# mic-rud/Learned-Compression-of-Point-Cloud-Geometry-and-Attributes

Hardware: AMD Instinct MI355X
Metric: encode+decode Mpoints/sec (higher is better)
Workload: dtype f32

## Files before the change

### learned-compression-of-point-cloud-geometry-and-attributes_amd/csrc/select.hip

```cpp
#include <stdlib.h>

#include "common.h"
#include "sort_small.h"

namespace pcc {

constexpr int TK_STRIDE = 264;
constexpr int TK_LDS_BATCHES = 16;

__device__ __forceinline__ uint32_t float_key(float v) {
    if (v != v) return 0xFFFFFFFFu;
    if (v == 0.0f) v = 0.0f;
    const uint32_t u = __float_as_uint(v);
    return (u & 0x80000000u) ? ~u : (u | 0x80000000u);
}

struct Key96 { uint32_t w[3]; };

__device__ __forceinline__ Key96 make_key(float logit, int4 c) {
    const uint64_t lo = ~pack_key(c.x, c.y, c.z, c.w);
    Key96 k;
    k.w[0] = float_key(logit);
    k.w[1] = (uint32_t)(lo >> 32);
    k.w[2] = (uint32_t)lo;
// ... 201 lines not shown

__global__ __launch_bounds__(256) void topk_write_mask(const float* __restrict__ logits, int ld,
                                                       const int32_t* __restrict__ coords, int64_t n, int nbatch,
                                                       const int32_t* __restrict__ state, uint8_t* __restrict__ mask) {
    const int64_t i = (int64_t)blockIdx.x * 256 + threadIdx.x;
    if (i >= n) return;
    const int4 c = reinterpret_cast<const int4*>(coords)[i];
    const int b = c.x;
    uint8_t m = 0;
    if (b >= 0 && b < nbatch) {
        const int32_t* st = state + (int64_t)b * TK_STRIDE;
        const int nb = st[2];
        if (nb <= 12) m = cmp_prefix(make_key(logits[i * ld], c), st, nb) >= 0 ? 1 : 0;
    }
    mask[i] = m;
}

constexpr int TK_SMALL_N = 32768;
__global__ __launch_bounds__(1024) void topk_small_kernel(const float* __restrict__ logits, int ld, const int32_t* __restrict__ coords, int n,
                                                          const int32_t* __restrict__ k, uint8_t* __restrict__ mask,
                                                          int32_t* __restrict__ state) {
    __shared__ int32_t st[8];
    __shared__ int h[256];
    __shared__ int total_s;
    const int t = threadIdx.x;
    if (t < 8) st[t] = 0;
    __syncthreads();
    if (t == 0) {
        const int kk = k[0];
        st[0] = kk;
        if (kk <= 0) { st[1] = 1; st[2] = 13; }
    }
    __syncthreads();
    for (int pass = 0; pass < 12; ++pass) {
        if (st[1]) break;
        if (t < 256) h[t] = 0;
        __syncthreads();
        const bool logit_only = pass < 4;
        for (int i = t; i < n; i += 1024) {
            const int4 c = logit_only ? make_int4(0, 0, 0, 0) : reinterpret_cast<const int4*>(coords)[i];
            if (c.x != 0) continue;
            const Key96 key = make_key(logits[(int64_t)i * ld], c);
            if (cmp_prefix(key, st, pass) != 0) continue;
            atomicAdd(&h[(key.w[pass >> 2] >> (8 * (3 - (pass & 3)))) & 0xFFu], 1);
        }
        __syncthreads();
        const int krem = st[0];
        int above = 0, mine = 0;
        if (t < 256) {
            mine = h[t];
            for (int j = t + 1; j < 256; ++j) above += h[j];
            if (t == 0) total_s = above + mine;
        }
        __syncthreads();
        if (pass == 0 && total_s <= krem) {
            if (t == 0) { st[1] = 1; st[2] = 0; }
        } else if (t < 256 && above < krem && krem <= above + mine) {
            const int word = pass >> 2, shift = 8 * (3 - (pass & 3));
            st[3 + word] = (int32_t)((uint32_t)st[3 + word] | ((uint32_t)t << shift));
            const int knew = krem - above;
            st[0] = knew;
            if (mine == knew || pass == 11) { st[1] = 1; st[2] = pass + 1; }
        }
        __syncthreads();
    }
    const int nb = st[2];
    for (int i = t; i < n; i += 1024) {
        const int4 c = reinterpret_cast<const int4*>(coords)[i];
        uint8_t m = 0;
        if (c.x == 0 && nb <= 12) m = cmp_prefix(make_key(logits[(int64_t)i * ld], c), st, nb) >= 0 ? 1 : 0;
        mask[i] = m;
    }
    for (int i = t; i < TK_STRIDE; i += 1024) state[i] = i < 8 ? st[i] : 0;
}

__global__ __launch_bounds__(256) void coords_to_keys(const int32_t* __restrict__ coords, int64_t n,
                                                      uint64_t* __restrict__ keys) {
    const int64_t i = (int64_t)blockIdx.x * 256 + threadIdx.x;
    if (i >= n) return;
    const int4 c = reinterpret_cast<const int4*>(coords)[i];
    keys[i] = pack_key(c.x, c.y, c.z, c.w);
}

__global__ __launch_bounds__(256) void mask_bit_counts_kernel(const uint32_t* __restrict__ row_mask, int64_t n,
                                                              uint32_t* __restrict__ counts) {
    __shared__ unsigned c[27];
    if (threadIdx.x < 27) c[threadIdx.x] = 0u;
    __syncthreads();
    unsigned mine[27];
#pragma unroll
    for (int b = 0; b < 27; ++b) mine[b] = 0u;
    for (int64_t i0 = (int64_t)blockIdx.x * 256; i0 < n; i0 += (int64_t)gridDim.x * 256) {
        const int64_t i = i0 + threadIdx.x;
        const uint32_t m = (i < n) ? row_mask[i] : 0u;
#pragma unroll
        for (int b = 0; b < 27; ++b) mine[b] += (unsigned)__popcll(__ballot((m >> b) & 1u));
    }
    if ((threadIdx.x & 63) == 0) {
#pragma unroll
        for (int b = 0; b < 27; ++b)
            if (mine[b]) atomicAdd(&c[b], mine[b]);
    }
    __syncthreads();
    if (threadIdx.x < 27 && c[threadIdx.x]) atomicAdd(&counts[threadIdx.x], c[threadIdx.x]);
}

__device__ __forceinline__ void order_bit_positions(const uint32_t* __restrict__ counts, int* pos_s) {
    if (threadIdx.x < 27) {
        const uint32_t mine = counts[threadIdx.x];
        int rank = 0;
        for (int b = 0; b < 27; ++b) {
            const uint32_t o = counts[b];
            rank += (o < mine || (o == mine && b < (int)threadIdx.x)) ? 1 : 0;
        }
        pos_s[threadIdx.x] = 26 - rank;
    }
    __syncthreads();
}

__device__ __forceinline__ uint32_t order_key_of(uint32_t m, const int* pos_s) {
    uint32_t key = 0u;
#pragma unroll
    for (int b = 0; b < 27; ++b) key |= ((m >> b) & 1u) << pos_s[b];
    return 0x7FFFFFFu - key;
}

__global__ __launch_bounds__(256) void order_keys32_kernel(const uint32_t* __restrict__ row_mask, int64_t n,
                                                           const uint32_t* __restrict__ counts, uint32_t* __restrict__ keys) {
    __shared__ int pos_s[27];
    order_bit_positions(counts, pos_s);
    const int64_t i = (int64_t)blockIdx.x * 256 + threadIdx.x;
    if (i >= n) return;
    const uint32_t m = row_mask[i] & 0x7FFFFFFu;
    keys[i] = order_key_of(m, pos_s);
}

__global__ __launch_bounds__(256) void order_keys64_kernel(const uint32_t* __restrict__ row_mask,
                                                           const int32_t* __restrict__ coords, int64_t n,
                                                           int block_log2, int ts, const uint32_t* __restrict__ counts,
                                                           uint64_t* __restrict__ keys) {
    __shared__ int pos_s[27];
    order_bit_positions(counts, pos_s);
    const int64_t i = (int64_t)blockIdx.x * 256 + threadIdx.x;
    if (i >= n) return;
    uint64_t key = order_key_of(row_mask[i] & 0x7FFFFFFu, pos_s);
    const int4 c = reinterpret_cast<const int4*>(coords)[i];
    const uint64_t bx = (uint64_t)(((c.y / ts) + 512) >> block_log2) & 0x3FF;
    const uint64_t by = (uint64_t)(((c.z / ts) + 512) >> block_log2) & 0x3FF;
    const uint64_t bz = (uint64_t)(((c.w / ts) + 512) >> block_log2) & 0x3FF;
    key |= ((((uint64_t)(c.x & 0x3) << 30) | (bx << 20) | (by << 10) | bz) << 32);
    keys[i] = key;
}

__global__ __launch_bounds__(256) void group_masks_kernel(const int32_t* __restrict__ order, const uint32_t* __restrict__ row_mask,
                                                          int64_t n, uint32_t* __restrict__ group_mask32) {
    const int64_t i = (int64_t)blockIdx.x * 256 + threadIdx.x;
    uint32_t m = (i < n) ? row_mask[order[i]] : 0u;
#pragma unroll
    for (int d = 1; d < 32; d <<= 1) m |= __shfl_xor(m, d, 64);
    if (i < n && (threadIdx.x & 31) == 0) group_mask32[i >> 5] = m;
}

__global__ __launch_bounds__(256) void permute_rows_kernel(const int32_t* __restrict__ order, const int32_t* __restrict__ nbr,
                                                           int64_t n, int K, int32_t* __restrict__ nbr_sorted) {
    __shared__ int32_t src_row[256];
    const int64_t r0 = (int64_t)blockIdx.x * 256;
    const int64_t i = r0 + threadIdx.x;
    src_row[threadIdx.x] = (i < n) ? order[i] : 0;
    __syncthreads();
    const int rows = (int)((n - r0 < 256) ? (n - r0) : 256);
    const int total = rows * K;
    int32_t* dst = nbr_sorted + r0 * K;
    for (int e = threadIdx.x; e < total; e += 256) {
        const int lr = e / K;
        const int k = e - lr * K;
        dst[e] = nbr[(int64_t)src_row[lr] * K + k];
    }
}


template <int ROUNDS>
__global__ __launch_bounds__(RS_SMALL_THREADS) void order_small_kernel(const uint32_t* __restrict__ row_mask, int n, uint32_t* keys_a,
                                                                      uint32_t* keys_b, int32_t* va, int32_t* vb) {
    __shared__ unsigned cnt27[27];
    __shared__ int pos_s[27];
    const int t = threadIdx.x;
    if (t < 27) cnt27[t] = 0u;
    __syncthreads();
    unsigned mine[27];
#pragma unroll
    for (int b = 0; b < 27; ++b) mine[b] = 0u;
    for (int i = t; i < n; i += RS_SMALL_THREADS) {
        const uint32_t m = row_mask[i];
#pragma unroll
        for (int b = 0; b < 27; ++b) mine[b] += (m >> b) & 1u;
    }
#pragma unroll
    for (int b = 0; b < 27; ++b) {
        unsigned v = mine[b];
#pragma unroll
        for (int d = 32; d >= 1; d >>= 1) v += __shfl_xor(v, d, 64);
        if ((t & 63) == 0 && v) atomicAdd(&cnt27[b], v);
    }
    __syncthreads();
    order_bit_positions(cnt27, pos_s);
    for (int i = t; i < n; i += RS_SMALL_THREADS) keys_a[i] = order_key_of(row_mask[i] & 0x7FFFFFFu, pos_s);
    __syncthreads();
    radix_sort_small_body<uint32_t, ROUNDS, 9>(keys_a, keys_b, va, vb, 1, n, 0, 27, 3);
}

constexpr int SMALL_MAP_MAX = 256;

template <int ROUNDS, int KS>
__global__ __launch_bounds__(RS_SMALL_THREADS) void small_map_kernel(const int32_t* __restrict__ out_coords, int n,
                                                                    const uint64_t* __restrict__ keys, const int32_t* __restrict__ vals,
                                                                    uint64_t tmask, int tshift, int step, int pitch,
                                                                    int32_t* nbr, uint32_t* __restrict__ row_mask, int32_t* order,
// ... 83 lines not shown
extern "C" {

int64_t pcc_small_map_max(void) {
    static int off = -1;
    if (off < 0) { const char* e = getenv("PCC_SMALL_MAP"); off = (e && e[0] == '0') ? 1 : 0; }
    return off ? 0 : SMALL_MAP_MAX;
}

int pcc_small_kernel_map(const int32_t* out_coords, int64_t n_out, const uint64_t* in_keys, const int32_t* in_vals, int64_t in_cap,
                         int32_t ksize, int32_t step, int32_t sign, int32_t* nbr, uint32_t* row_mask, int32_t* order,
                         uint32_t* group_mask32, void* scratch, int64_t scratch_bytes, void* stream) {
    PCC_REQUIRE(ksize == 2 || ksize == 3, "pcc_small_kernel_map: kernel size must be 2 or 3");
    PCC_REQUIRE(sign == 1 || sign == -1, "pcc_small_kernel_map: sign must be +1/-1");
    PCC_REQUIRE(in_cap > 0 && (in_cap & (in_cap - 1)) == 0, "pcc_small_kernel_map: bad capacity");
    PCC_REQUIRE(step >= 1, "pcc_small_kernel_map: step must be >= 1");
    PCC_REQUIRE(n_out >= 0 && n_out <= SMALL_MAP_MAX, "pcc_small_kernel_map: %lld rows exceed %d", (long long)n_out, SMALL_MAP_MAX);
    PCC_REQUIRE(scratch_bytes >= pcc_sort_scratch_bytes(n_out), "pcc_small_kernel_map: scratch too small");
    if (n_out <= 0) return PCC_OK;
    const int in_stride = sign > 0 ? step : 2 * step;
    const int pitch = sign > 0 ? 0 : 2 * step;
    char* p = reinterpret_cast<char*>(scratch);
    uint32_t* keys_a = reinterpret_cast<uint32_t*>(p); p += align256(n_out * 8);
    uint32_t* keys_b = reinterpret_cast<uint32_t*>(p); p += align256(n_out * 8);
    int32_t* vals_x = reinterpret_cast<int32_t*>(p);
    const int rounds = (int)(((n_out + RS_SMALL_WAVES - 1) / RS_SMALL_WAVES + 63) / 64);
    hipStream_t st = as_stream(stream);
#define PCC_SMALL_MAP(R, S)                                                                                                          \
    hipLaunchKernelGGL((small_map_kernel<R, S>), dim3(1), dim3(RS_SMALL_THREADS), 0, st, out_coords, (int)n_out, in_keys, in_vals,    \
                       (uint64_t)(in_cap - 1), grid_shift_of(in_stride), sign * step, pitch, nbr, row_mask, order,                   \
                       group_mask32, keys_a, keys_b, vals_x)
#define PCC_SMALL_MAP_R(S)                                                                                                           \
    do {                                                                                                                             \
        if (rounds <= 1) PCC_SMALL_MAP(1, S);                                                                                        \
        else if (rounds <= 2) PCC_SMALL_MAP(2, S);                                                                                   \
        else PCC_SMALL_MAP(4, S);                                                                                                    \
    } while (0)
    if (ksize == 3) PCC_SMALL_MAP_R(3);
    else PCC_SMALL_MAP_R(2);
#undef PCC_SMALL_MAP_R
#undef PCC_SMALL_MAP
    PCC_LAUNCH_CHECK();
    return PCC_OK;
}

int64_t pcc_topk_state_elems(int32_t nbatch) { return (int64_t)nbatch * TK_STRIDE + (nbatch == 1 ? (int64_t)TK1_GROUPS * 256 : 0); }

int pcc_topk_mask(const float* logits, int32_t ld, const int32_t* coords, int64_t n, int32_t nbatch, const int32_t* k,
                  uint8_t* mask, int32_t* state, void* stream) {
    PCC_REQUIRE(nbatch >= 1 && nbatch <= BATCH_LIMIT + 1, "pcc_topk_mask: bad nbatch %d", nbatch);
    PCC_REQUIRE(ld >= 1, "pcc_topk_mask: bad leading dimension");
    hipStream_t st = as_stream(stream);
    if (small_path_enabled(1) && nbatch == 1 && n > 0 && n <= TK_SMALL_N) {
        hipLaunchKernelGGL(topk_small_kernel, dim3(1), dim3(1024), 0, st, logits, ld, coords, (int)n, k, mask, state);
        PCC_LAUNCH_CHECK();
        return PCC_OK;
    }
    hipLaunchKernelGGL(topk_init, dim3(nbatch), dim3(256), 0, st, k, nbatch, state);
    if (n > 0) {
        const unsigned nb = blocks_for(n, 256, 512);
        if (nbatch == 1 && small_path_enabled(1)) {
            const unsigned groups = blocks_for(n, TK1_THREADS * 4, TK1_GROUPS);
            int32_t* partial = state + TK_STRIDE;
            for (int pass = 0; pass < 4; ++pass) {
                hipLaunchKernelGGL(topk_hist1_kernel, dim3(groups), dim3(TK1_THREADS), 0, st, logits, ld, n, pass, state, partial);
                hipLaunchKernelGGL(topk_pick1_kernel, dim3(1), dim3(1024), 0, st, pass, state, partial, (int)groups);
            }
            hipLaunchKernelGGL(topk_tail_kernel, dim3(1), dim3(1024), 0, st, logits, ld, coords, n, state);
            hipLaunchKernelGGL(topk_write_mask, dim3(blocks_for(n, 256)), dim3(256), 0, st, logits, ld, coords, n, nbatch,
                               state, mask);
            PCC_LAUNCH_CHECK();
            return PCC_OK;
        }
        for (int pass = 0; pass < 12; ++pass) {
            hipLaunchKernelGGL(topk_hist, dim3(nb), dim3(256), 0, st, logits, ld, coords, n, nbatch, pass, state);
            hipLaunchKernelGGL(topk_pick, dim3(nbatch), dim3(256), 0, st, pass, state);
        }
        hipLaunchKernelGGL(topk_write_mask, dim3(blocks_for(n, 256)), dim3(256), 0, st, logits, ld, coords, n, nbatch,
                           state, mask);
    }
    PCC_LAUNCH_CHECK();
    return PCC_OK;
}

int64_t pcc_order_scratch_bytes(int64_t n) { return pcc_sort_scratch_bytes(n); }

int pcc_order_rows_by_mask(const uint32_t* row_mask, const int32_t* coords, int64_t n, int32_t block_log2,
                           int32_t tensor_stride, int32_t* order, uint32_t* group_mask32, void* scratch, int64_t scratch_bytes,
                           void* stream) {
    if (n <= 0) return PCC_OK;
    PCC_REQUIRE(n < (1ll << 31), "pcc_order_rows_by_mask: too many rows");
    PCC_REQUIRE(block_log2 < 0 || coords != nullptr, "pcc_order_rows_by_mask: block ordering needs coordinates");
    PCC_REQUIRE(block_log2 <= 10, "pcc_order_rows_by_mask: block_log2 out of range");
    PCC_REQUIRE(tensor_stride >= 1, "pcc_order_rows_by_mask: bad tensor stride");
    PCC_REQUIRE(scratch_bytes >= pcc_sort_scratch_bytes(n), "pcc_order_rows_by_mask: scratch too small");
    hipStream_t st = as_stream(stream);
    char* p = reinterpret_cast<char*>(scratch);
    char* keys_a = p; p += align256(n * 8);
    char* keys_b = p; p += align256(n * 8);
    int32_t* vals_x = reinterpret_cast<int32_t*>(p); p += align256(n * 4);
    void* counters = p;
    uint32_t* bit_counts = reinterpret_cast<uint32_t*>(p + radix_sort_counter_bytes(n));
    if (small_path_enabled(0) && block_log2 < 0 && n <= RS_SMALL_N) {
        const int rounds = (int)(((n + RS_SMALL_WAVES - 1) / RS_SMALL_WAVES + 63) / 64);
        uint32_t* ka = reinterpret_cast<uint32_t*>(keys_a);
        uint32_t* kb = reinterpret_cast<uint32_t*>(keys_b);
#define PCC_ORDER_SMALL(R) hipLaunchKernelGGL(order_small_kernel<R>, dim3(1), dim3(RS_SMALL_THREADS), 0, st, row_mask, (int)n, ka, kb, vals_x, order)
        if (rounds <= 1) PCC_ORDER_SMALL(1);
        else if (rounds <= 2) PCC_ORDER_SMALL(2);
        else if (rounds <= 4) PCC_ORDER_SMALL(4);
        else if (rounds <= 8) PCC_ORDER_SMALL(8);
        else PCC_ORDER_SMALL(16);
#undef PCC_ORDER_SMALL
        hipLaunchKernelGGL(group_masks_kernel, dim3(blocks_for(n, 256)), dim3(256), 0, st, order, row_mask, n, group_mask32);
        PCC_LAUNCH_CHECK();
        return PCC_OK;
    }
    PCC_CHECK_HIP(hipMemsetAsync(bit_counts, 0, 27 * sizeof(uint32_t), st));
    hipLaunchKernelGGL(mask_bit_counts_kernel, dim3(blocks_for(n, 256 * 16, 512)), dim3(256), 0, st, row_mask, n, bit_counts);
    const int begin = 0, end = block_log2 >= 0 ? 64 : 27;
    const int digit_bits = block_log2 >= 0 ? 8 : radix_sort_order_digit_bits(n);
    const bool in_b = radix_sort_result_in_b(begin, end, digit_bits);
    int32_t* va = in_b ? vals_x : order;
    int32_t* vb = in_b ? order : vals_x;
    int rc;
    if (block_log2 < 0) {
        hipLaunchKernelGGL(order_keys32_kernel, dim3(blocks_for(n, 256)), dim3(256), 0, st, row_mask, n, bit_counts,
                           reinterpret_cast<uint32_t*>(keys_a));
        rc = radix_sort_pairs_u32(reinterpret_cast<uint32_t*>(keys_a), reinterpret_cast<uint32_t*>(keys_b), va, vb, true, n, begin, end,
                                  counters, st, digit_bits);
    } else {
        hipLaunchKernelGGL(order_keys64_kernel, dim3(blocks_for(n, 256)), dim3(256), 0, st, row_mask, coords, n, block_log2, tensor_stride,
                           bit_counts, reinterpret_cast<uint64_t*>(keys_a));
        rc = radix_sort_pairs_u64(reinterpret_cast<uint64_t*>(keys_a), reinterpret_cast<uint64_t*>(keys_b), va, vb, true, n, begin, end,
                                  counters, st);
    }
    if (rc) return rc;
    hipLaunchKernelGGL(group_masks_kernel, dim3(blocks_for(n, 256)), dim3(256), 0, st, order, row_mask, n, group_mask32);
    PCC_LAUNCH_CHECK();
    return PCC_OK;
}

int pcc_permute_map_rows(const int32_t* nbr, const int32_t* order, int64_t n, int32_t K, int32_t* nbr_sorted, void* stream) {
    PCC_REQUIRE(K >= 1 && K <= 27, "pcc_permute_map_rows: K out of range");
    PCC_REQUIRE(nbr != nullptr && order != nullptr && nbr_sorted != nullptr, "pcc_permute_map_rows: null argument");
    if (n <= 0) return PCC_OK;
    hipLaunchKernelGGL(permute_rows_kernel, dim3(blocks_for(n, 256)), dim3(256), 0, as_stream(stream), order, nbr, n, K, nbr_sorted);
    PCC_LAUNCH_CHECK();
    return PCC_OK;
}

int64_t pcc_sort_scratch_bytes(int64_t n) {
    if (n < 1) n = 1;
    return 2 * align256(n * 8) + align256(n * 4) + radix_sort_counter_bytes(n) + 256;
}

int pcc_sort_coords(const int32_t* coords, int64_t n, int32_t* perm, void* scratch, int64_t scratch_bytes, void* stream) {
    if (n <= 0) return PCC_OK;
    PCC_REQUIRE(n < (1ll << 31), "pcc_sort_coords: too many rows");
    PCC_REQUIRE(scratch_bytes >= pcc_sort_scratch_bytes(n), "pcc_sort_coords: scratch too small");
    hipStream_t st = as_stream(stream);
    char* p = reinterpret_cast<char*>(scratch);
    uint64_t* keys_a = reinterpret_cast<uint64_t*>(p); p += align256(n * 8);
    uint64_t* keys_b = reinterpret_cast<uint64_t*>(p); p += align256(n * 8);
    int32_t* vals_x = reinterpret_cast<int32_t*>(p); p += align256(n * 4);
    void* counters = p;
    hipLaunchKernelGGL(coords_to_keys, dim3(blocks_for(n, 256)), dim3(256), 0, st, coords, n, keys_a);
    const bool in_b = radix_sort_result_in_b(0, 64);
    return radix_sort_pairs_u64(keys_a, keys_b, in_b ? vals_x : perm, in_b ? perm : vals_x, true, n, 0, 64, counters, st);
}

}
```

### learned-compression-of-point-cloud-geometry-and-attributes_amd/csrc/sort.h

```cpp
#pragma once
#include "common.h"

namespace pcc {

static inline int64_t align256(int64_t v) { return (v + 255) / 256 * 256; }

int64_t scan_block_sums_elems(int64_t m);
int scan_flags(const int32_t* flags, int64_t m, int32_t* pos, int32_t* block_sums, int64_t* total, int inclusive,
               hipStream_t st, const int32_t* err = nullptr);

int radix_sort_passes(int begin_bit, int end_bit, int digit_bits = 8);
static inline bool radix_sort_result_in_b(int begin_bit, int end_bit, int digit_bits = 8) { return radix_sort_passes(begin_bit, end_bit, digit_bits) & 1; }
int64_t radix_sort_counter_bytes(int64_t n);
int radix_sort_order_digit_bits(int64_t n);
int radix_sort_pairs_u32(uint32_t* keys_a, uint32_t* keys_b, int32_t* vals_a, int32_t* vals_b, bool vals_are_iota, int64_t n,
                         int begin_bit, int end_bit, void* counters, hipStream_t st, int digit_bits = 8);
int radix_sort_pairs_u64(uint64_t* keys_a, uint64_t* keys_b, int32_t* vals_a, int32_t* vals_b, bool vals_are_iota, int64_t n,
                         int begin_bit, int end_bit, void* counters, hipStream_t st);

}
```

### learned-compression-of-point-cloud-geometry-and-attributes_amd/csrc/sort.hip

```cpp
#include "sort_small.h"

namespace pcc {

constexpr int RS_MID_ITEMS = 8;
constexpr int RS_MID_MAX_UNITS = 64;
constexpr int RS_BIG_ITEMS = 16;

template <class K, int ROUNDS, int DB>
__global__ __launch_bounds__(RS_SMALL_THREADS) void radix_sort_small_kernel(K* ka, K* kb, int32_t* va, int32_t* vb, int iota, int n,
                                                                           int begin_bit, int end_bit, int passes) {
    radix_sort_small_body<K, ROUNDS, DB>(ka, kb, va, vb, iota, n, begin_bit, end_bit, passes);
}

template <class K, int ITEMS, int DB>
__global__ __launch_bounds__(256) void radix_count_kernel(const K* __restrict__ keys, int64_t n, int shift, unsigned dmask,
                                                          int64_t nunits, int32_t* __restrict__ counts) {
    constexpr int ND = 1 << DB;
    __shared__ int cnt[ND];
#pragma unroll
    for (int d = threadIdx.x; d < ND; d += 256) cnt[d] = 0;
    __syncthreads();
    const int64_t base = (int64_t)blockIdx.x * (256 * ITEMS);
    K key[ITEMS];
#pragma unroll
    for (int j = 0; j < ITEMS; ++j) {
        const int64_t i = base + (int64_t)j * 256 + threadIdx.x;
        key[j] = (i < n) ? keys[i] : (K)0;
    }
#pragma unroll
    for (int j = 0; j < ITEMS; ++j)
        if (base + (int64_t)j * 256 + threadIdx.x < n) atomicAdd(&cnt[(unsigned)(key[j] >> shift) & dmask], 1);
    __syncthreads();
#pragma unroll
    for (int d = threadIdx.x; d < ND; d += 256) counts[(int64_t)d * nunits + blockIdx.x] = cnt[d];
}

__global__ __launch_bounds__(256) void radix_rowscan_kernel(int32_t* __restrict__ counts, int64_t nunits, int32_t* __restrict__ totals) {
    __shared__ int wsum[4];
    __shared__ int carry_s;
    const int t = threadIdx.x, lane = t & 63, w = t >> 6;
    int32_t* row = counts + (int64_t)blockIdx.x * nunits;
    if (t == 0) carry_s = 0;
    __syncthreads();
    for (int64_t base = 0; base < nunits; base += 1024) {
        const int64_t i = base + 4 * (int64_t)t;
        int f[4];
        int v = 0;
#pragma unroll
        for (int j = 0; j < 4; ++j) {
            f[j] = (i + j < nunits) ? row[i + j] : 0;
            v += f[j];
        }
        const int inc = wave_inclusive_scan_i32(v, lane);
        if (lane == 63) wsum[w] = inc;
        __syncthreads();
        int pre = carry_s;
        for (int ww = 0; ww < w; ++ww) pre += wsum[ww];
        int ex = pre + inc - v;
#pragma unroll
        for (int j = 0; j < 4; ++j) {
            if (i + j < nunits) row[i + j] = ex;
            ex += f[j];
        }
        __syncthreads();
        if (t == 255) carry_s = pre + inc;
        __syncthreads();
    }
    if (t == 0) totals[blockIdx.x] = carry_s;
}

template <class K, int ITEMS, bool SELF_PREFIX, int DB>
__global__ __launch_bounds__(256) void radix_scatter_kernel(const K* __restrict__ src, K* __restrict__ dst, const int32_t* __restrict__ vs,
                                                            int32_t* __restrict__ vd, int iota, int64_t n, int shift, unsigned dmask,
                                                            int64_t nunits, const int32_t* __restrict__ counts,
                                                            const int32_t* __restrict__ totals) {
    constexpr int WAVE_KEYS = 64 * ITEMS, WG_KEYS = 4 * WAVE_KEYS;
    constexpr int ND = 1 << DB, DH = ND / 256;
    __shared__ K skey[WG_KEYS];
    __shared__ int32_t sval[WG_KEYS];
    __shared__ int cnt[4][ND];
    __shared__ int lbase[ND];
    __shared__ int gbase[ND];
    __shared__ int wsum[4], wsum2[4];
    const int t = threadIdx.x, lane = t & 63, w = t >> 6;
    const uint64_t lt = (1ull << lane) - 1ull;
    for (int i = t; i < 4 * ND; i += 256) (&cnt[0][0])[i] = 0;
    const int64_t base0 = (int64_t)blockIdx.x * WG_KEYS;
    const int64_t wbase = base0 + (int64_t)w * WAVE_KEYS;
    K key[ITEMS];
    int32_t val[ITEMS];
#pragma unroll
    for (int j = 0; j < ITEMS; ++j) {
        const int64_t i = wbase + j * 64 + lane;
        key[j] = (i < n) ? src[i] : (K)0;
        val[j] = (i < n) ? (iota ? (int32_t)i : vs[i]) : 0;
    }
    int pre[DH], total[DH];
#pragma unroll
    for (int h = 0; h < DH; ++h) {
        const int d = h * 256 + t;
        if (SELF_PREFIX) {
            const int32_t* row = counts + (int64_t)d * nunits;
            pre[h] = 0;
            total[h] = 0;
            for (int64_t u = 0; u < nunits; ++u) {
                const int c = row[u];
                total[h] += c;
                pre[h] += (u < (int64_t)blockIdx.x) ? c : 0;
            }
        } else {
            pre[h] = counts[(int64_t)d * nunits + blockIdx.x];
            total[h] = totals[d];
        }
    }
    __syncthreads();
#pragma unroll
    for (int j = 0; j < ITEMS; ++j)
        if (wbase + j * 64 + lane < n) atomicAdd(&cnt[w][(unsigned)(key[j] >> shift) & dmask], 1);
    __syncthreads();
    int gcarry = 0, lcarry = 0;
#pragma unroll
    for (int h = 0; h < DH; ++h) {
        const int d = h * 256 + t;
        const int c0 = cnt[0][d], c1 = cnt[1][d], c2 = cnt[2][d], c3 = cnt[3][d];
        const int mine = c0 + c1 + c2 + c3;
        const int inc = wave_inclusive_scan_i32(total[h], lane);
        const int linc = wave_inclusive_scan_i32(mine, lane);
        if (lane == 63) { wsum[w] = inc; wsum2[w] = linc; }
        __syncthreads();
        int run = gcarry + pre[h] + inc - total[h], lrun = lcarry + linc - mine;
        for (int ww = 0; ww < w; ++ww) { run += wsum[ww]; lrun += wsum2[ww]; }
        gcarry += wsum[0] + wsum[1] + wsum[2] + wsum[3];
        lcarry += wsum2[0] + wsum2[1] + wsum2[2] + wsum2[3];
        gbase[d] = run;
        lbase[d] = lrun;
        cnt[0][d] = lrun;
        cnt[1][d] = lrun + c0;
        cnt[2][d] = lrun + c0 + c1;
        cnt[3][d] = lrun + c0 + c1 + c2;
        __syncthreads();
    }
#pragma unroll
    for (int j = 0; j < ITEMS; ++j) {
        const bool active = wbase + j * 64 + lane < n;
        const unsigned d = (unsigned)(key[j] >> shift) & dmask;
        const uint64_t same = match_digit<DB>(d, active);
        const int below = __popcll(same & lt);
        int base = 0;
        if (active) {
            base = cnt[w][d];
            skey[base + below] = key[j];
            sval[base + below] = val[j];
        }
        __builtin_amdgcn_wave_barrier();
        if (active && below == 0) cnt[w][d] = base + __popcll(same);
        __builtin_amdgcn_wave_barrier();
    }
    __syncthreads();
    const int nk = (int)((n - base0 < WG_KEYS) ? (n - base0) : WG_KEYS);
    for (int i = t; i < nk; i += 256) {
        const K k = skey[i];
        const unsigned d = (unsigned)(k >> shift) & dmask;
        const int64_t pos = (int64_t)gbase[d] + (i - lbase[d]);
        dst[pos] = k;
        vd[pos] = sval[i];
    }
}

int radix_sort_passes(int begin_bit, int end_bit, int digit_bits) {
    return end_bit > begin_bit ? (end_bit - begin_bit + digit_bits - 1) / digit_bits : 0;
}

int radix_sort_order_digit_bits(int64_t n) {
    const int64_t mid_units = (n + 256 * RS_MID_ITEMS - 1) / (256 * RS_MID_ITEMS);
    return (n > RS_SMALL_N && mid_units <= RS_MID_MAX_UNITS) ? 8 : 9;
}

int64_t radix_sort_counter_bytes(int64_t n) {
    const int64_t mid = (n + 256 * RS_MID_ITEMS - 1) / (256 * RS_MID_ITEMS), big = (n + 256 * RS_BIG_ITEMS - 1) / (256 * RS_BIG_ITEMS);
    const int64_t nunits = mid <= RS_MID_MAX_UNITS ? mid : big;
    return align256(512 * (nunits > 0 ? nunits : 1) * 4) + 2048;
}

template <class K, int DB>
static int radix_sort_pairs(K* ka, K* kb, int32_t* va, int32_t* vb, bool iota, int64_t n, int begin_bit, int end_bit, void* counters,
                            hipStream_t st) {
    constexpr int ND = 1 << DB;
    const int passes = radix_sort_passes(begin_bit, end_bit, DB);
    PCC_REQUIRE(passes >= 1 && end_bit <= (int)(8 * sizeof(K)) && begin_bit >= 0, "radix sort: bad bit range [%d, %d)", begin_bit, end_bit);
    PCC_REQUIRE(n < (1ll << 31), "radix sort: too many keys (%lld)", (long long)n);
    if (n <= 0) return PCC_OK;
    if (n <= RS_SMALL_N) {
        const int rounds = (int)(((n + RS_SMALL_WAVES - 1) / RS_SMALL_WAVES + 63) / 64);
#define PCC_RS_SMALL(R)                                                                                                             \
    hipLaunchKernelGGL((radix_sort_small_kernel<K, R, DB>), dim3(1), dim3(RS_SMALL_THREADS), 0, st, ka, kb, va, vb, iota ? 1 : 0, (int)n, \
                       begin_bit, end_bit, passes)
        if (rounds <= 1) PCC_RS_SMALL(1);
        else if (rounds <= 2) PCC_RS_SMALL(2);
        else if (rounds <= 4) PCC_RS_SMALL(4);
        else if (rounds <= 8) PCC_RS_SMALL(8);
        else PCC_RS_SMALL(16);
#undef PCC_RS_SMALL
        PCC_LAUNCH_CHECK();
        return PCC_OK;
    }
    const int64_t mid_units = (n + 256 * RS_MID_ITEMS - 1) / (256 * RS_MID_ITEMS);
    const bool mid = mid_units <= RS_MID_MAX_UNITS;
    const int64_t nunits = mid ? mid_units : (n + 256 * RS_BIG_ITEMS - 1) / (256 * RS_BIG_ITEMS);
    int32_t* counts = reinterpret_cast<int32_t*>(counters);
    int32_t* totals = counts + align256((int64_t)ND * nunits * 4) / 4;
    K* src = ka;
    K* dst = kb;
    int32_t* vs = va;
    int32_t* vd = vb;
    for (int p = 0; p < passes; ++p) {
        const int shift = begin_bit + DB * p;
        const unsigned dmask = (end_bit - shift >= DB) ? (unsigned)(ND - 1) : ((1u << (end_bit - shift)) - 1u);
        const int io = (iota && p == 0) ? 1 : 0;
        if (mid) {
            hipLaunchKernelGGL((radix_count_kernel<K, RS_MID_ITEMS, DB>), dim3((unsigned)nunits), dim3(256), 0, st, src, n, shift, dmask, nunits, counts);
            hipLaunchKernelGGL((radix_scatter_kernel<K, RS_MID_ITEMS, true, DB>), dim3((unsigned)nunits), dim3(256), 0, st, src, dst, vs, vd, io, n,
                               shift, dmask, nunits, counts, totals);
        } else {
            hipLaunchKernelGGL((radix_count_kernel<K, RS_BIG_ITEMS, DB>), dim3((unsigned)nunits), dim3(256), 0, st, src, n, shift, dmask, nunits, counts);
            hipLaunchKernelGGL(radix_rowscan_kernel, dim3(ND), dim3(256), 0, st, counts, nunits, totals);
            hipLaunchKernelGGL((radix_scatter_kernel<K, RS_BIG_ITEMS, false, DB>), dim3((unsigned)nunits), dim3(256), 0, st, src, dst, vs, vd, io, n,
                               shift, dmask, nunits, counts, totals);
        }
        K* tk = src; src = dst; dst = tk;
        int32_t* tv = vs; vs = vd; vd = tv;
    }
    PCC_LAUNCH_CHECK();
    return PCC_OK;
}

int radix_sort_pairs_u32(uint32_t* keys_a, uint32_t* keys_b, int32_t* vals_a, int32_t* vals_b, bool vals_are_iota, int64_t n, int begin_bit,
                         int end_bit, void* counters, hipStream_t st, int digit_bits) {
    if (digit_bits == 9) return radix_sort_pairs<uint32_t, 9>(keys_a, keys_b, vals_a, vals_b, vals_are_iota, n, begin_bit, end_bit, counters, st);
    return radix_sort_pairs<uint32_t, 8>(keys_a, keys_b, vals_a, vals_b, vals_are_iota, n, begin_bit, end_bit, counters, st);
}

int radix_sort_pairs_u64(uint64_t* keys_a, uint64_t* keys_b, int32_t* vals_a, int32_t* vals_b, bool vals_are_iota, int64_t n, int begin_bit,
                         int end_bit, void* counters, hipStream_t st) {
    return radix_sort_pairs<uint64_t, 8>(keys_a, keys_b, vals_a, vals_b, vals_are_iota, n, begin_bit, end_bit, counters, st);
}

}
```

### learned-compression-of-point-cloud-geometry-and-attributes_amd/csrc/sort_small.h

```cpp
#pragma once
#include "sort.h"

namespace pcc {

constexpr int RS_SMALL_THREADS = 1024;
constexpr int RS_SMALL_WAVES = RS_SMALL_THREADS / 64;
constexpr int RS_SMALL_ROUNDS = 16;
constexpr int64_t RS_SMALL_N = (int64_t)RS_SMALL_WAVES * 64 * RS_SMALL_ROUNDS;

template <int DB = 8>
__device__ __forceinline__ uint64_t match_digit(unsigned d, bool active) {
    uint64_t same = __ballot(active);
#pragma unroll
    for (int b = 0; b < DB; ++b) {
        const bool bit = (d >> b) & 1u;
        const uint64_t bal = __ballot(active && bit);
        same &= bit ? bal : ~bal;
    }
    return same;
}

__device__ __forceinline__ int wave_inclusive_scan_i32(int v, int lane) {
#pragma unroll
    for (int d = 1; d < 64; d <<= 1) {
        const int t = __shfl_up(v, d, 64);
        if (lane >= d) v += t;
    }
    return v;
}

template <class K, int ROUNDS, int DB = 8>
__device__ __forceinline__ void radix_sort_small_body(K* ka, K* kb, int32_t* va, int32_t* vb, int iota, int n, int begin_bit, int end_bit,
                                                      int passes) {
    constexpr int ND = 1 << DB;
    static_assert(ND <= RS_SMALL_THREADS, "one thread per digit");
    __shared__ int cnt[RS_SMALL_WAVES][ND];
    __shared__ int tot[ND];
    __shared__ int wsum[ND / 64];
    const int t = threadIdx.x, lane = t & 63, w = t >> 6;
    const int chunk = ((n + RS_SMALL_WAVES - 1) / RS_SMALL_WAVES + 63) / 64 * 64;
    const int lo = w * chunk < n ? w * chunk : n;
    const int hi = lo + chunk < n ? lo + chunk : n;
    const uint64_t lt = (1ull << lane) - 1ull;
    K* src = ka;
    K* dst = kb;
    int32_t* vs = va;
    int32_t* vd = vb;
    for (int p = 0; p < passes; ++p) {
        const int shift = begin_bit + DB * p;
        const unsigned dmask = (end_bit - shift >= DB) ? (unsigned)(ND - 1) : ((1u << (end_bit - shift)) - 1u);
        K key[ROUNDS];
        int32_t val[ROUNDS];
#pragma unroll
        for (int j = 0; j < ROUNDS; ++j) {
            const int i = lo + j * 64 + lane;
            key[j] = (i < hi) ? src[i] : (K)0;
            val[j] = (i < hi) ? ((iota && p == 0) ? i : vs[i]) : 0;
        }
        for (int i = t; i < RS_SMALL_WAVES * ND; i += RS_SMALL_THREADS) (&cnt[0][0])[i] = 0;
        __syncthreads();
#pragma unroll
        for (int j = 0; j < ROUNDS; ++j)
            if (lo + j * 64 + lane < hi) atomicAdd(&cnt[w][(unsigned)(key[j] >> shift) & dmask], 1);
        __syncthreads();
        int v = 0;
        if (t < ND) {
            int run = 0;
#pragma unroll
            for (int ww = 0; ww < RS_SMALL_WAVES; ++ww) {
                const int c = cnt[ww][t];
                cnt[ww][t] = run;
                run += c;
            }
            v = run;
        }
        const int inc = wave_inclusive_scan_i32(v, lane);
        if (lane == 63 && w < ND / 64) wsum[w] = inc;
        __syncthreads();
        if (t < ND) {
            int base = 0;
            for (int ww = 0; ww < w; ++ww) base += wsum[ww];
            tot[t] = base + inc - v;
        }
        __syncthreads();
#pragma unroll
        for (int j = 0; j < ROUNDS; ++j) {
            const int i = lo + j * 64 + lane;
            const bool active = i < hi;
            const unsigned d = (unsigned)(key[j] >> shift) & dmask;
            const uint64_t same = match_digit<DB>(d, active);
            const int below = __popcll(same & lt);
            int base = 0;
            if (active) {
                base = cnt[w][d];
                const int pos = tot[d] + base + below;
                dst[pos] = key[j];
                vd[pos] = val[j];
            }
            __builtin_amdgcn_wave_barrier();
            if (active && below == 0) cnt[w][d] = base + __popcll(same);
            __builtin_amdgcn_wave_barrier();
        }
        __syncthreads();
        K* tk = src; src = dst; dst = tk;
        int32_t* tv = vs; vs = vd; vd = tv;
    }
}

}
```

Baseline: 8.888.

## Build distinct-mask rank table to collapse order radix sort to one pass

While counting mask bits, each block inserts distinct row masks into an LDS hash table and then into a global one. The last block to finish computes bit positions and, when there are few distinct masks, assigns each one a dense rank. The first radix pass now computes keys straight from row_mask, so the separate key-building kernel goes away. When the rank table applies, the two remaining passes return immediately through a device-side skip flag. This trades extra atomics and hash probing in the count kernel, plus a last-block ticket protocol, for fewer sort passes. The full three-pass sort still runs when masks are highly distinct.

```diff
diff --git a/learned-compression-of-point-cloud-geometry-and-attributes_amd/csrc/select.hip b/learned-compression-of-point-cloud-geometry-and-attributes_amd/csrc/select.hip
--- a/learned-compression-of-point-cloud-geometry-and-attributes_amd/csrc/select.hip
+++ b/learned-compression-of-point-cloud-geometry-and-attributes_amd/csrc/select.hip
@@ -307,10 +307,34 @@
     keys[i] = pack_key(c.x, c.y, c.z, c.w);
 }
 
+constexpr int ORDER_LOCAL_SLOTS = 1024;
+
+__device__ __forceinline__ void order_plan_insert(OrderPlan* plan, uint32_t v) {
+    unsigned h = order_tab_hash(v);
+    for (int probe = 0; probe < ORDER_TAB_SLOTS; ++probe) {
+        if ((probe & 7) == 0 && __hip_atomic_load(&plan->ndistinct, __ATOMIC_RELAXED, __HIP_MEMORY_SCOPE_AGENT) > (uint32_t)ORDER_FEW_KEYS) return;
+        uint32_t cur = __hip_atomic_load(&plan->tab[h], __ATOMIC_RELAXED, __HIP_MEMORY_SCOPE_AGENT);
+        if (cur == 0u) {
+            cur = atomicCAS(&plan->tab[h], 0u, v);
+            if (cur == 0u) { atomicAdd(&plan->ndistinct, 1u); return; }
+        }
+        if (cur == v) return;
+        h = (h + 1) & (ORDER_TAB_SLOTS - 1);
+    }
+    atomicAdd(&plan->ndistinct, (uint32_t)ORDER_FEW_KEYS + 1u);
+}
+
+template <bool PLAN>
 __global__ __launch_bounds__(256) void mask_bit_counts_kernel(const uint32_t* __restrict__ row_mask, int64_t n,
-                                                              uint32_t* __restrict__ counts) {
+                                                              uint32_t* __restrict__ counts, OrderPlan* plan) {
     __shared__ unsigned c[27];
+    __shared__ uint32_t ltab[PLAN ? ORDER_LOCAL_SLOTS : 1];
+    __shared__ unsigned lcount;
     if (threadIdx.x < 27) c[threadIdx.x] = 0u;
+    if constexpr (PLAN) {
+        for (int i = threadIdx.x; i < ORDER_LOCAL_SLOTS; i += 256) ltab[i] = 0u;
+        if (threadIdx.x == 0) lcount = 0u;
+    }
     __syncthreads();
     unsigned mine[27];
 #pragma unroll
@@ -320,6 +344,25 @@
         const uint32_t m = (i < n) ? row_mask[i] : 0u;
 #pragma unroll
         for (int b = 0; b < 27; ++b) mine[b] += (unsigned)__popcll(__ballot((m >> b) & 1u));
+        if constexpr (PLAN) {
+            if (i < n && __hip_atomic_load(&lcount, __ATOMIC_RELAXED, __HIP_MEMORY_SCOPE_WORKGROUP) <= (unsigned)ORDER_FEW_KEYS) {
+                const uint32_t v = (m & 0x7FFFFFFu) + 1u;
+                unsigned h = order_tab_hash(v) & (ORDER_LOCAL_SLOTS - 1);
+                for (int probe = 0; probe < ORDER_LOCAL_SLOTS; ++probe) {
+                    uint32_t cur = __hip_atomic_load(&ltab[h], __ATOMIC_RELAXED, __HIP_MEMORY_SCOPE_WORKGROUP);
+                    if (cur == 0u) {
+                        cur = atomicCAS(&ltab[h], 0u, v);
+                        if (cur == 0u) {
+                            atomicAdd(&lcount, 1u);
+                            order_plan_insert(plan, v);
+                            break;
+                        }
+                    }
+                    if (cur == v) break;
+                    h = (h + 1) & (ORDER_LOCAL_SLOTS - 1);
+                }
+            }
+        }
     }
     if ((threadIdx.x & 63) == 0) {
 #pragma unroll
@@ -328,36 +371,53 @@
     }
     __syncthreads();
     if (threadIdx.x < 27 && c[threadIdx.x]) atomicAdd(&counts[threadIdx.x], c[threadIdx.x]);
-}
-
-__device__ __forceinline__ void order_bit_positions(const uint32_t* __restrict__ counts, int* pos_s) {
-    if (threadIdx.x < 27) {
-        const uint32_t mine = counts[threadIdx.x];
-        int rank = 0;
-        for (int b = 0; b < 27; ++b) {
-            const uint32_t o = counts[b];
-            rank += (o < mine || (o == mine && b < (int)threadIdx.x)) ? 1 : 0;
-        }
-        pos_s[threadIdx.x] = 26 - rank;
-    }
-    __syncthreads();
-}
-
-__device__ __forceinline__ uint32_t order_key_of(uint32_t m, const int* pos_s) {
-    uint32_t key = 0u;
-#pragma unroll
-    for (int b = 0; b < 27; ++b) key |= ((m >> b) & 1u) << pos_s[b];
-    return 0x7FFFFFFu - key;
-}
-
-__global__ __launch_bounds__(256) void order_keys32_kernel(const uint32_t* __restrict__ row_mask, int64_t n,
-                                                           const uint32_t* __restrict__ counts, uint32_t* __restrict__ keys) {
-    __shared__ int pos_s[27];
-    order_bit_positions(counts, pos_s);
-    const int64_t i = (int64_t)blockIdx.x * 256 + threadIdx.x;
-    if (i >= n) return;
-    const uint32_t m = row_mask[i] & 0x7FFFFFFu;
-    keys[i] = order_key_of(m, pos_s);
+    if constexpr (PLAN) {
+        __shared__ int last_s, nk_s;
+        __shared__ unsigned cnt_s[27];
+        __shared__ int pos_s[27];
+        __shared__ uint32_t key_s[ORDER_FEW_KEYS];
+        __shared__ int slot_s[ORDER_FEW_KEYS];
+        if (lcount > (unsigned)ORDER_FEW_KEYS && threadIdx.x == 0) atomicAdd(&plan->ndistinct, (uint32_t)ORDER_FEW_KEYS + 1u);
+        asm volatile("s_waitcnt vmcnt(0)" ::: "memory");
+        __syncthreads();
+        if (threadIdx.x == 0) {
+            __builtin_amdgcn_fence(__ATOMIC_RELEASE, "agent");
+            asm volatile("s_waitcnt vmcnt(0)" ::: "memory");
+            last_s = __hip_atomic_fetch_add(&plan->ticket, 1u, __ATOMIC_RELAXED, __HIP_MEMORY_SCOPE_AGENT) == gridDim.x - 1 ? 1 : 0;
+            nk_s = 0;
+        }
+        __syncthreads();
+        if (!last_s) return;
+        __builtin_amdgcn_fence(__ATOMIC_ACQUIRE, "agent");
+        if (threadIdx.x < 27) cnt_s[threadIdx.x] = atomicAdd(&counts[threadIdx.x], 0u);
+        __syncthreads();
+        order_bit_positions(cnt_s, pos_s);
+        if (threadIdx.x < 27) plan->pos[threadIdx.x] = pos_s[threadIdx.x];
+        if (threadIdx.x == 0) {
+            last_s = atomicAdd(&plan->ndistinct, 0u) <= (uint32_t)ORDER_FEW_KEYS ? 1 : 0;
+            plan->few = last_s;
+        }
+        __syncthreads();
+        if (!last_s) return;
+        for (int sl = threadIdx.x; sl < ORDER_TAB_SLOTS; sl += 256) {
+            const uint32_t v = atomicOr(&plan->tab[sl], 0u);
+            if (v != 0u) {
+                const int e = atomicAdd(&nk_s, 1);
+                if (e < ORDER_FEW_KEYS) {
+                    key_s[e] = order_key_of(v - 1u, pos_s);
+                    slot_s[e] = sl;
+                }
+            }
+        }
+        __syncthreads();
+        const int nk = nk_s < ORDER_FEW_KEYS ? nk_s : ORDER_FEW_KEYS;
+        for (int e = threadIdx.x; e < nk; e += 256) {
+            const uint32_t k = key_s[e];
+            int r = 0;
+            for (int j = 0; j < nk; ++j) r += key_s[j] < k ? 1 : 0;
+            plan->rank[slot_s[e]] = r;
+        }
+    }
 }
 
 __global__ __launch_bounds__(256) void order_keys64_kernel(const uint32_t* __restrict__ row_mask,
@@ -607,7 +667,7 @@
     return PCC_OK;
 }
 
-int64_t pcc_order_scratch_bytes(int64_t n) { return pcc_sort_scratch_bytes(n); }
+int64_t pcc_order_scratch_bytes(int64_t n) { return pcc_sort_scratch_bytes(n) + align256((int64_t)sizeof(OrderPlan)); }
 
 int pcc_order_rows_by_mask(const uint32_t* row_mask, const int32_t* coords, int64_t n, int32_t block_log2,
                            int32_t tensor_stride, int32_t* order, uint32_t* group_mask32, void* scratch, int64_t scratch_bytes,
@@ -617,14 +677,15 @@
     PCC_REQUIRE(block_log2 < 0 || coords != nullptr, "pcc_order_rows_by_mask: block ordering needs coordinates");
     PCC_REQUIRE(block_log2 <= 10, "pcc_order_rows_by_mask: block_log2 out of range");
     PCC_REQUIRE(tensor_stride >= 1, "pcc_order_rows_by_mask: bad tensor stride");
-    PCC_REQUIRE(scratch_bytes >= pcc_sort_scratch_bytes(n), "pcc_order_rows_by_mask: scratch too small");
+    PCC_REQUIRE(scratch_bytes >= pcc_order_scratch_bytes(n), "pcc_order_rows_by_mask: scratch too small");
     hipStream_t st = as_stream(stream);
     char* p = reinterpret_cast<char*>(scratch);
     char* keys_a = p; p += align256(n * 8);
     char* keys_b = p; p += align256(n * 8);
     int32_t* vals_x = reinterpret_cast<int32_t*>(p); p += align256(n * 4);
     void* counters = p;
-    uint32_t* bit_counts = reinterpret_cast<uint32_t*>(p + radix_sort_counter_bytes(n));
+    OrderPlan* plan = reinterpret_cast<OrderPlan*>(p + radix_sort_counter_bytes(n));
+    uint32_t* bit_counts = plan->bit_counts;
     if (small_path_enabled(0) && block_log2 < 0 && n <= RS_SMALL_N) {
         const int rounds = (int)(((n + RS_SMALL_WAVES - 1) / RS_SMALL_WAVES + 63) / 64);
         uint32_t* ka = reinterpret_cast<uint32_t*>(keys_a);
@@ -640,24 +701,20 @@
         PCC_LAUNCH_CHECK();
         return PCC_OK;
     }
-    PCC_CHECK_HIP(hipMemsetAsync(bit_counts, 0, 27 * sizeof(uint32_t), st));
-    hipLaunchKernelGGL(mask_bit_counts_kernel, dim3(blocks_for(n, 256 * 16, 512)), dim3(256), 0, st, row_mask, n, bit_counts);
-    const int begin = 0, end = block_log2 >= 0 ? 64 : 27;
-    const int digit_bits = block_log2 >= 0 ? 8 : radix_sort_order_digit_bits(n);
-    const bool in_b = radix_sort_result_in_b(begin, end, digit_bits);
-    int32_t* va = in_b ? vals_x : order;
-    int32_t* vb = in_b ? order : vals_x;
     int rc;
     if (block_log2 < 0) {
-        hipLaunchKernelGGL(order_keys32_kernel, dim3(blocks_for(n, 256)), dim3(256), 0, st, row_mask, n, bit_counts,
-                           reinterpret_cast<uint32_t*>(keys_a));
-        rc = radix_sort_pairs_u32(reinterpret_cast<uint32_t*>(keys_a), reinterpret_cast<uint32_t*>(keys_b), va, vb, true, n, begin, end,
-                                  counters, st, digit_bits);
+        PCC_CHECK_HIP(hipMemsetAsync(plan, 0, offsetof(OrderPlan, rank), st));
+        hipLaunchKernelGGL(mask_bit_counts_kernel<true>, dim3(blocks_for(n, 256 * 16, 512)), dim3(256), 0, st, row_mask, n, bit_counts, plan);
+        rc = radix_sort_order_u32(row_mask, plan, reinterpret_cast<uint32_t*>(keys_a), reinterpret_cast<uint32_t*>(keys_b), vals_x, order, n,
+                                  counters, st);
     } else {
+        PCC_CHECK_HIP(hipMemsetAsync(bit_counts, 0, 27 * sizeof(uint32_t), st));
+        hipLaunchKernelGGL(mask_bit_counts_kernel<false>, dim3(blocks_for(n, 256 * 16, 512)), dim3(256), 0, st, row_mask, n, bit_counts, plan);
+        const bool in_b = radix_sort_result_in_b(0, 64);
         hipLaunchKernelGGL(order_keys64_kernel, dim3(blocks_for(n, 256)), dim3(256), 0, st, row_mask, coords, n, block_log2, tensor_stride,
                            bit_counts, reinterpret_cast<uint64_t*>(keys_a));
-        rc = radix_sort_pairs_u64(reinterpret_cast<uint64_t*>(keys_a), reinterpret_cast<uint64_t*>(keys_b), va, vb, true, n, begin, end,
-                                  counters, st);
+        rc = radix_sort_pairs_u64(reinterpret_cast<uint64_t*>(keys_a), reinterpret_cast<uint64_t*>(keys_b), in_b ? vals_x : order,
+                                  in_b ? order : vals_x, true, n, 0, 64, counters, st);
     }
     if (rc) return rc;
     hipLaunchKernelGGL(group_masks_kernel, dim3(blocks_for(n, 256)), dim3(256), 0, st, order, row_mask, n, group_mask32);
diff --git a/learned-compression-of-point-cloud-geometry-and-attributes_amd/csrc/sort.h b/learned-compression-of-point-cloud-geometry-and-attributes_amd/csrc/sort.h
--- a/learned-compression-of-point-cloud-geometry-and-attributes_amd/csrc/sort.h
+++ b/learned-compression-of-point-cloud-geometry-and-attributes_amd/csrc/sort.h
@@ -12,10 +12,14 @@
 int radix_sort_passes(int begin_bit, int end_bit, int digit_bits = 8);
 static inline bool radix_sort_result_in_b(int begin_bit, int end_bit, int digit_bits = 8) { return radix_sort_passes(begin_bit, end_bit, digit_bits) & 1; }
 int64_t radix_sort_counter_bytes(int64_t n);
-int radix_sort_order_digit_bits(int64_t n);
 int radix_sort_pairs_u32(uint32_t* keys_a, uint32_t* keys_b, int32_t* vals_a, int32_t* vals_b, bool vals_are_iota, int64_t n,
                          int begin_bit, int end_bit, void* counters, hipStream_t st, int digit_bits = 8);
 int radix_sort_pairs_u64(uint64_t* keys_a, uint64_t* keys_b, int32_t* vals_a, int32_t* vals_b, bool vals_are_iota, int64_t n,
                          int begin_bit, int end_bit, void* counters, hipStream_t st);
 
+
+struct OrderPlan;
+int radix_sort_order_u32(const uint32_t* row_mask, const OrderPlan* plan, uint32_t* keys_a, uint32_t* keys_b, int32_t* vals_x,
+                         int32_t* order, int64_t n, void* counters, hipStream_t st);
+
 }
diff --git a/learned-compression-of-point-cloud-geometry-and-attributes_amd/csrc/sort.hip b/learned-compression-of-point-cloud-geometry-and-attributes_amd/csrc/sort.hip
--- a/learned-compression-of-point-cloud-geometry-and-attributes_amd/csrc/sort.hip
+++ b/learned-compression-of-point-cloud-geometry-and-attributes_amd/csrc/sort.hip
@@ -12,11 +12,26 @@
     radix_sort_small_body<K, ROUNDS, DB>(ka, kb, va, vb, iota, n, begin_bit, end_bit, passes);
 }
 
-template <class K, int ITEMS, int DB>
+__device__ __forceinline__ uint32_t order_first_key(uint32_t mask, int few, const OrderPlan* __restrict__ plan, const int* pos_s) {
+    const uint32_t m = mask & 0x7FFFFFFu;
+    return few ? order_rank_of(plan, m) : order_key_of(m, pos_s);
+}
+
+template <class K, int ITEMS, int DB, bool FROM_MASK>
 __global__ __launch_bounds__(256) void radix_count_kernel(const K* __restrict__ keys, int64_t n, int shift, unsigned dmask,
-                                                          int64_t nunits, int32_t* __restrict__ counts) {
+                                                          int64_t nunits, int32_t* __restrict__ counts,
+                                                          const uint32_t* __restrict__ row_mask, const OrderPlan* __restrict__ plan,
+                                                          const int32_t* __restrict__ skip) {
     constexpr int ND = 1 << DB;
     __shared__ int cnt[ND];
+    __shared__ int pos_s[27];
+    int few = 0;
+    if constexpr (FROM_MASK) {
+        few = plan->few;
+        if (threadIdx.x < 27) pos_s[threadIdx.x] = plan->pos[threadIdx.x];
+    } else {
+        if (skip != nullptr && *skip != 0) return;
+    }
 #pragma unroll
     for (int d = threadIdx.x; d < ND; d += 256) cnt[d] = 0;
     __syncthreads();
@@ -25,7 +40,8 @@
 #pragma unroll
     for (int j = 0; j < ITEMS; ++j) {
         const int64_t i = base + (int64_t)j * 256 + threadIdx.x;
-        key[j] = (i < n) ? keys[i] : (K)0;
+        if constexpr (FROM_MASK) key[j] = (i < n) ? (K)order_first_key(row_mask[i], few, plan, pos_s) : (K)0;
+        else key[j] = (i < n) ? keys[i] : (K)0;
     }
 #pragma unroll
     for (int j = 0; j < ITEMS; ++j)
@@ -35,9 +51,11 @@
     for (int d = threadIdx.x; d < ND; d += 256) counts[(int64_t)d * nunits + blockIdx.x] = cnt[d];
 }
 
-__global__ __launch_bounds__(256) void radix_rowscan_kernel(int32_t* __restrict__ counts, int64_t nunits, int32_t* __restrict__ totals) {
+__global__ __launch_bounds__(256) void radix_rowscan_kernel(int32_t* __restrict__ counts, int64_t nunits, int32_t* __restrict__ totals,
+                                                            const int32_t* __restrict__ skip) {
     __shared__ int wsum[4];
     __shared__ int carry_s;
+    if (skip != nullptr && *skip != 0) return;
     const int t = threadIdx.x, lane = t & 63, w = t >> 6;
     int32_t* row = counts + (int64_t)blockIdx.x * nunits;
     if (t == 0) carry_s = 0;
@@ -69,11 +87,12 @@
     if (t == 0) totals[blockIdx.x] = carry_s;
 }
 
-template <class K, int ITEMS, bool SELF_PREFIX, int DB>
+template <class K, int ITEMS, bool SELF_PREFIX, int DB, bool FROM_MASK>
 __global__ __launch_bounds__(256) void radix_scatter_kernel(const K* __restrict__ src, K* __restrict__ dst, const int32_t* __restrict__ vs,
                                                             int32_t* __restrict__ vd, int iota, int64_t n, int shift, unsigned dmask,
                                                             int64_t nunits, const int32_t* __restrict__ counts,
-                                                            const int32_t* __restrict__ totals) {
+                                                            const int32_t* __restrict__ totals, const uint32_t* __restrict__ row_mask,
+                                                            const OrderPlan* __restrict__ plan, const int32_t* __restrict__ skip) {
     constexpr int WAVE_KEYS = 64 * ITEMS, WG_KEYS = 4 * WAVE_KEYS;
     constexpr int ND = 1 << DB, DH = ND / 256;
     __shared__ K skey[WG_KEYS];
@@ -82,8 +101,17 @@
     __shared__ int lbase[ND];
     __shared__ int gbase[ND];
     __shared__ int wsum[4], wsum2[4];
+    __shared__ int pos_s[27];
     const int t = threadIdx.x, lane = t & 63, w = t >> 6;
     const uint64_t lt = (1ull << lane) - 1ull;
+    int few = 0;
+    if constexpr (FROM_MASK) {
+        few = plan->few;
+        if (t < 27) pos_s[t] = plan->pos[t];
+        __syncthreads();
+    } else {
+        if (skip != nullptr && *skip != 0) return;
+    }
     for (int i = t; i < 4 * ND; i += 256) (&cnt[0][0])[i] = 0;
     const int64_t base0 = (int64_t)blockIdx.x * WG_KEYS;
     const int64_t wbase = base0 + (int64_t)w * WAVE_KEYS;
@@ -92,7 +120,8 @@
 #pragma unroll
     for (int j = 0; j < ITEMS; ++j) {
         const int64_t i = wbase + j * 64 + lane;
-        key[j] = (i < n) ? src[i] : (K)0;
+        if constexpr (FROM_MASK) key[j] = (i < n) ? (K)order_first_key(row_mask[i], few, plan, pos_s) : (K)0;
+        else key[j] = (i < n) ? src[i] : (K)0;
         val[j] = (i < n) ? (iota ? (int32_t)i : vs[i]) : 0;
     }
     int pre[DH], total[DH];
@@ -162,18 +191,13 @@
         const K k = skey[i];
         const unsigned d = (unsigned)(k >> shift) & dmask;
         const int64_t pos = (int64_t)gbase[d] + (i - lbase[d]);
-        dst[pos] = k;
+        if (!FROM_MASK || !few) dst[pos] = k;
         vd[pos] = sval[i];
     }
 }
 
 int radix_sort_passes(int begin_bit, int end_bit, int digit_bits) {
     return end_bit > begin_bit ? (end_bit - begin_bit + digit_bits - 1) / digit_bits : 0;
-}
-
-int radix_sort_order_digit_bits(int64_t n) {
-    const int64_t mid_units = (n + 256 * RS_MID_ITEMS - 1) / (256 * RS_MID_ITEMS);
-    return (n > RS_SMALL_N && mid_units <= RS_MID_MAX_UNITS) ? 8 : 9;
 }
 
 int64_t radix_sort_counter_bytes(int64_t n) {
@@ -213,19 +237,24 @@
     K* dst = kb;
     int32_t* vs = va;
     int32_t* vd = vb;
+    const uint32_t* nomask = nullptr;
+    const OrderPlan* noplan = nullptr;
+    const int32_t* noskip = nullptr;
     for (int p = 0; p < passes; ++p) {
         const int shift = begin_bit + DB * p;
         const unsigned dmask = (end_bit - shift >= DB) ? (unsigned)(ND - 1) : ((1u << (end_bit - shift)) - 1u);
         const int io = (iota && p == 0) ? 1 : 0;
         if (mid) {
-            hipLaunchKernelGGL((radix_count_kernel<K, RS_MID_ITEMS, DB>), dim3((unsigned)nunits), dim3(256), 0, st, src, n, shift, dmask, nunits, counts);
-            hipLaunchKernelGGL((radix_scatter_kernel<K, RS_MID_ITEMS, true, DB>), dim3((unsigned)nunits), dim3(256), 0, st, src, dst, vs, vd, io, n,
-                               shift, dmask, nunits, counts, totals);
+            hipLaunchKernelGGL((radix_count_kernel<K, RS_MID_ITEMS, DB, false>), dim3((unsigned)nunits), dim3(256), 0, st, src, n, shift, dmask, nunits,
+                               counts, nomask, noplan, noskip);
+            hipLaunchKernelGGL((radix_scatter_kernel<K, RS_MID_ITEMS, true, DB, false>), dim3((unsigned)nunits), dim3(256), 0, st, src, dst, vs, vd, io, n,
+                               shift, dmask, nunits, counts, totals, nomask, noplan, noskip);
         } else {
-            hipLaunchKernelGGL((radix_count_kernel<K, RS_BIG_ITEMS, DB>), dim3((unsigned)nunits), dim3(256), 0, st, src, n, shift, dmask, nunits, counts);
-            hipLaunchKernelGGL(radix_rowscan_kernel, dim3(ND), dim3(256), 0, st, counts, nunits, totals);
-            hipLaunchKernelGGL((radix_scatter_kernel<K, RS_BIG_ITEMS, false, DB>), dim3((unsigned)nunits), dim3(256), 0, st, src, dst, vs, vd, io, n,
-                               shift, dmask, nunits, counts, totals);
+            hipLaunchKernelGGL((radix_count_kernel<K, RS_BIG_ITEMS, DB, false>), dim3((unsigned)nunits), dim3(256), 0, st, src, n, shift, dmask, nunits,
+                               counts, nomask, noplan, noskip);
+            hipLaunchKernelGGL(radix_rowscan_kernel, dim3(ND), dim3(256), 0, st, counts, nunits, totals, noskip);
+            hipLaunchKernelGGL((radix_scatter_kernel<K, RS_BIG_ITEMS, false, DB, false>), dim3((unsigned)nunits), dim3(256), 0, st, src, dst, vs, vd, io, n,
+                               shift, dmask, nunits, counts, totals, nomask, noplan, noskip);
         }
         K* tk = src; src = dst; dst = tk;
         int32_t* tv = vs; vs = vd; vd = tv;
@@ -240,6 +269,53 @@
     return radix_sort_pairs<uint32_t, 8>(keys_a, keys_b, vals_a, vals_b, vals_are_iota, n, begin_bit, end_bit, counters, st);
 }
 
+int radix_sort_order_u32(const uint32_t* row_mask, const OrderPlan* plan, uint32_t* keys_a, uint32_t* keys_b, int32_t* vals_x,
+                         int32_t* order, int64_t n, void* counters, hipStream_t st) {
+    constexpr int DB = 9, ND = 1 << DB;
+    PCC_REQUIRE(n < (1ll << 31), "radix sort: too many keys (%lld)", (long long)n);
+    if (n <= 0) return PCC_OK;
+    const int64_t mid_units = (n + 256 * RS_MID_ITEMS - 1) / (256 * RS_MID_ITEMS);
+    const bool mid = mid_units <= RS_MID_MAX_UNITS;
+    const int64_t nunits = mid ? mid_units : (n + 256 * RS_BIG_ITEMS - 1) / (256 * RS_BIG_ITEMS);
+    int32_t* counts = reinterpret_cast<int32_t*>(counters);
+    int32_t* totals = counts + align256((int64_t)ND * nunits * 4) / 4;
+    const dim3 grid((unsigned)nunits), block(256);
+    const unsigned dmask = ND - 1;
+    const uint32_t* nokeys = nullptr;
+    const int32_t* novals = nullptr;
+    const int32_t* noskip = nullptr;
+    const int32_t* few = &plan->few;
+    if (mid) {
+        hipLaunchKernelGGL((radix_count_kernel<uint32_t, RS_MID_ITEMS, DB, true>), grid, block, 0, st, nokeys, n, 0, dmask, nunits, counts, row_mask, plan, noskip);
+        hipLaunchKernelGGL((radix_scatter_kernel<uint32_t, RS_MID_ITEMS, true, DB, true>), grid, block, 0, st, nokeys, keys_b, novals, order, 1, n, 0, dmask,
+                           nunits, counts, totals, row_mask, plan, noskip);
+    } else {
+        hipLaunchKernelGGL((radix_count_kernel<uint32_t, RS_BIG_ITEMS, DB, true>), grid, block, 0, st, nokeys, n, 0, dmask, nunits, counts, row_mask, plan, noskip);
+        hipLaunchKernelGGL(radix_rowscan_kernel, dim3(ND), block, 0, st, counts, nunits, totals, noskip);
+        hipLaunchKernelGGL((radix_scatter_kernel<uint32_t, RS_BIG_ITEMS, false, DB, true>), grid, block, 0, st, nokeys, keys_b, novals, order, 1, n, 0, dmask,
+                           nunits, counts, totals, row_mask, plan, noskip);
+    }
+    for (int p = 1; p < 3; ++p) {
+        const int shift = DB * p;
+        const uint32_t* src = p == 1 ? keys_b : keys_a;
+        uint32_t* dst = p == 1 ? keys_a : keys_b;
+        const int32_t* vs = p == 1 ? order : vals_x;
+        int32_t* vd = p == 1 ? vals_x : order;
+        if (mid) {
+            hipLaunchKernelGGL((radix_count_kernel<uint32_t, RS_MID_ITEMS, DB, false>), grid, block, 0, st, src, n, shift, dmask, nunits, counts, row_mask, plan, few);
+            hipLaunchKernelGGL((radix_scatter_kernel<uint32_t, RS_MID_ITEMS, true, DB, false>), grid, block, 0, st, src, dst, vs, vd, 0, n, shift, dmask,
+                               nunits, counts, totals, row_mask, plan, few);
+        } else {
+            hipLaunchKernelGGL((radix_count_kernel<uint32_t, RS_BIG_ITEMS, DB, false>), grid, block, 0, st, src, n, shift, dmask, nunits, counts, row_mask, plan, few);
+            hipLaunchKernelGGL(radix_rowscan_kernel, dim3(ND), block, 0, st, counts, nunits, totals, few);
+            hipLaunchKernelGGL((radix_scatter_kernel<uint32_t, RS_BIG_ITEMS, false, DB, false>), grid, block, 0, st, src, dst, vs, vd, 0, n, shift, dmask,
+                               nunits, counts, totals, row_mask, plan, few);
+        }
+    }
+    PCC_LAUNCH_CHECK();
+    return PCC_OK;
+}
+
 int radix_sort_pairs_u64(uint64_t* keys_a, uint64_t* keys_b, int32_t* vals_a, int32_t* vals_b, bool vals_are_iota, int64_t n, int begin_bit,
                          int end_bit, void* counters, hipStream_t st) {
     return radix_sort_pairs<uint64_t, 8>(keys_a, keys_b, vals_a, vals_b, vals_are_iota, n, begin_bit, end_bit, counters, st);
diff --git a/learned-compression-of-point-cloud-geometry-and-attributes_amd/csrc/sort_small.h b/learned-compression-of-point-cloud-geometry-and-attributes_amd/csrc/sort_small.h
--- a/learned-compression-of-point-cloud-geometry-and-attributes_amd/csrc/sort_small.h
+++ b/learned-compression-of-point-cloud-geometry-and-attributes_amd/csrc/sort_small.h
@@ -27,6 +27,50 @@
         if (lane >= d) v += t;
     }
     return v;
+}
+
+__device__ __forceinline__ void order_bit_positions(const uint32_t* __restrict__ counts, int* pos_s) {
+    if (threadIdx.x < 27) {
+        const uint32_t mine = counts[threadIdx.x];
+        int rank = 0;
+        for (int b = 0; b < 27; ++b) {
+            const uint32_t o = counts[b];
+            rank += (o < mine || (o == mine && b < (int)threadIdx.x)) ? 1 : 0;
+        }
+        pos_s[threadIdx.x] = 26 - rank;
+    }
+    __syncthreads();
+}
+
+__device__ __forceinline__ uint32_t order_key_of(uint32_t m, const int* pos_s) {
+    uint32_t key = 0u;
+#pragma unroll
+    for (int b = 0; b < 27; ++b) key |= ((m >> b) & 1u) << pos_s[b];
+    return 0x7FFFFFFu - key;
+}
+
+constexpr int ORDER_FEW_KEYS = 512;
+constexpr int ORDER_TAB_SLOTS = 2048;
+struct OrderPlan {
+    uint32_t bit_counts[27];
+    uint32_t ndistinct;
+    uint32_t ticket;
+    int32_t few;
+    int32_t pos[27];
+    uint32_t tab[ORDER_TAB_SLOTS];
+    int32_t rank[ORDER_TAB_SLOTS];
+};
+
+__device__ __forceinline__ unsigned order_tab_hash(uint32_t v) { return (v * 0x9E3779B1u) >> 21; }
+
+__device__ __forceinline__ uint32_t order_rank_of(const OrderPlan* __restrict__ plan, uint32_t m) {
+    const uint32_t v = m + 1u;
+    unsigned h = order_tab_hash(v);
+    for (int probe = 0; probe < ORDER_TAB_SLOTS; ++probe) {
+        if (plan->tab[h] == v) return (uint32_t)plan->rank[h];
+        h = (h + 1) & (ORDER_TAB_SLOTS - 1);
+    }
+    return 0u;
 }
 
 template <class K, int ROUNDS, int DB = 8>
```

New measurement: 8.717. 0.981x the previous value.
